# tlk00/BitMagic

Measured on AMD Instinct MI355X. Metric: Gbits/s + % HBM roofline, 256-way fused AND+COUNT on 1B-bit vectors, higher is better.
Workload: dtype u64; 1 GPU; aggregator pipeline combine_and_sub counts-only: 256-way AND+COUNT, 256 x 1000000000-bit vectors in total, data set A (common 10% OR noise 10%: no early exit); vectors=256, bits_per_vector=1000000000, density_q16=6554, blocks_per_vector=15259, blocks_per_rank=15259, hbm_resident_bytes=32279432448

## Files before the change

bitmagic_amd/csrc/bmx_device.h:

```cpp
#pragma once
#include <hip/hip_runtime.h>
#include <stdint.h>

typedef uint8_t  u8;
typedef uint16_t u16;
typedef uint32_t u32;
typedef uint64_t u64;

#define GMETA(e) ((u32)((e) >> 48) & 0x1FFFu)
#define GMETA_NONE 0xFFFFFFFFu
#define BMX_DESC_KIND(d) ((u32)((d) & 3ull))
#define BMX_DESC_PTR(d)  ((d) & ~3ull)

typedef u32 u32x4 __attribute__((ext_vector_type(4)));
typedef const __attribute__((address_space(1))) u32x4* gcptr4;
typedef __attribute__((address_space(1))) u32x4* gptr4;
typedef const __attribute__((address_space(1))) u16* gcptr16;

template <int ROWS> struct Part { u32x4 r[ROWS]; };
typedef Part<8> Blk;

__device__ __forceinline__ gcptr4 as_gc4(u64 addr) { return (gcptr4)(uintptr_t)addr; }
__device__ __forceinline__ gcptr4 as_gc4(const void* p) { return (gcptr4)(uintptr_t)p; }
__device__ __forceinline__ gptr4 as_g4(void* p) { return (gptr4)(uintptr_t)p; }
__device__ __forceinline__ gcptr16 as_gc16(u64 addr) { return (gcptr16)(uintptr_t)(addr & 0x0000FFFFFFFFFFFFull); }

__device__ __forceinline__ u32 lane_id() { return threadIdx.x & 63u; }

__device__ __forceinline__ u64 uniform64(u64 v)
{
    u32 lo = __builtin_amdgcn_readfirstlane((u32)v);
    u32 hi = __builtin_amdgcn_readfirstlane((u32)(v >> 32));
    return ((u64)hi << 32) | lo;
}
__device__ __forceinline__ u32 uniform32(u32 v) { return __builtin_amdgcn_readfirstlane(v); }

__device__ __forceinline__ u32 wave_sum(u32 v)
{
#pragma unroll
    for (int o = 32; o > 0; o >>= 1) v += __shfl_xor(v, o, 64);
    return v;
}

__device__ __forceinline__ u32 wave_scan_incl(u32 v, u32 )
{
    v += (u32)__builtin_amdgcn_update_dpp(0, (int)v, 0x111, 0xf, 0xf, false);
    v += (u32)__builtin_amdgcn_update_dpp(0, (int)v, 0x112, 0xf, 0xf, false);
    v += (u32)__builtin_amdgcn_update_dpp(0, (int)v, 0x114, 0xf, 0xf, false);
    v += (u32)__builtin_amdgcn_update_dpp(0, (int)v, 0x118, 0xf, 0xf, false);
    v += (u32)__builtin_amdgcn_update_dpp(0, (int)v, 0x142, 0xa, 0xf, false);
    v += (u32)__builtin_amdgcn_update_dpp(0, (int)v, 0x143, 0xc, 0xf, false);
    return v;
}

template <int ROWS, bool NT>
__device__ __forceinline__ void part_load(Part<ROWS>& b, gcptr4 p, u32 lane)
{
#pragma unroll
    for (int i = 0; i < ROWS; ++i) {
        if constexpr (NT) b.r[i] = __builtin_nontemporal_load(p + i * 64 + lane);
        else b.r[i] = p[i * 64 + lane];
    }
}
template <int ROWS>
__device__ __forceinline__ bool part_is_zero(const Part<ROWS>& b)
{
    u32 v = 0;
#pragma unroll
    for (int i = 0; i < ROWS; ++i) v |= b.r[i].x | b.r[i].y | b.r[i].z | b.r[i].w;
    return __ballot(v != 0u) == 0ull;
}
template <int ROWS>
__device__ __forceinline__ bool part_is_ones(const Part<ROWS>& b)
{
    u32 v = ~0u;
#pragma unroll
    for (int i = 0; i < ROWS; ++i) v &= b.r[i].x & b.r[i].y & b.r[i].z & b.r[i].w;
    return __ballot(v != ~0u) == 0ull;
}

__device__ __forceinline__ void blk_load(Blk& b, gcptr4 p, u32 lane)
{
#pragma unroll
    for (int i = 0; i < 8; ++i) b.r[i] = p[i * 64 + lane];
}
__device__ __forceinline__ void blk_store(const Blk& b, gptr4 p, u32 lane)
{
#pragma unroll
    for (int i = 0; i < 8; ++i) p[i * 64 + lane] = b.r[i];
}
__device__ __forceinline__ void blk_fill(Blk& b, u32 v)
{
#pragma unroll
    for (int i = 0; i < 8; ++i) b.r[i] = (u32x4)(v);
}
__device__ __forceinline__ void blk_and(Blk& a, const Blk& b)
{
#pragma unroll
    for (int i = 0; i < 8; ++i) a.r[i] &= b.r[i];
}
__device__ __forceinline__ void blk_andn(Blk& a, const Blk& b)
{
#pragma unroll
    for (int i = 0; i < 8; ++i) a.r[i] &= ~b.r[i];
}
__device__ __forceinline__ void blk_or(Blk& a, const Blk& b)
{
#pragma unroll
    for (int i = 0; i < 8; ++i) a.r[i] |= b.r[i];
}
__device__ __forceinline__ void blk_xor(Blk& a, const Blk& b)
{
#pragma unroll
    for (int i = 0; i < 8; ++i) a.r[i] ^= b.r[i];
}
__device__ __forceinline__ void blk_op(int op, Blk& a, const Blk& b)
{
    switch (op) { case 0: blk_and(a, b); break; case 1: blk_or(a, b); break;
                  case 2: blk_xor(a, b); break; default: blk_andn(a, b); break; }
}
__device__ __forceinline__ u32 blk_lane_or(const Blk& b)
{
    u32 v = 0;
#pragma unroll
    for (int i = 0; i < 8; ++i) v |= b.r[i].x | b.r[i].y | b.r[i].z | b.r[i].w;
    return v;
}
__device__ __forceinline__ u32 blk_lane_and(const Blk& b)
{
    u32 v = ~0u;
#pragma unroll
    for (int i = 0; i < 8; ++i) v &= b.r[i].x & b.r[i].y & b.r[i].z & b.r[i].w;
    return v;
}
// ... 604 lines not shown
```

bitmagic_amd/csrc/bmx_kernels6.h:

```cpp
#pragma once
#include "bmx_kernels5.h"


#define COLL_FLAG_FULL 1u
#define COLL_FLAG_NULL 2u
#define COLL_FLAG_BIT  4u
#define COLL_NGAP(f) ((f) >> 8)

typedef const __attribute__((address_space(1))) u64* coll_gc64;
typedef const __attribute__((address_space(1))) u32* coll_gc32;

__device__ __forceinline__ u32 coll_runs_of(u32 meta, u32 polarity)
{
    u32 len = meta >> 1, s = meta & 1u;
    u32 ones = s ? (len + 1u) >> 1 : len >> 1;
    return polarity ? ones : len - ones;
}

__global__ __launch_bounds__(256)
void k_coll_count(const u64* const* __restrict__ descs, const u32* __restrict__ nblk, u32 n, u32 ncols, u32 polarity,
                  u32* __restrict__ pre, u32* __restrict__ cnt, u32* __restrict__ flags)
{
    u32 c = blockIdx.x * blockDim.x + threadIdx.x;
    if (c >= ncols) return;
// ... 114 lines not shown
                for (int k = 0; k < 4; ++k) ns += (4u * q + (u32)k < m_cnt && p.start[k] == p.end[k]) ? 1u : 0u;
            }
        }
#pragma unroll
        for (u32 o = 1; o < (u32)L; o <<= 1) ns += __shfl_xor(ns, o, 64);
        if (in && t == 0) sgl[(size_t)i * ncols + c] = ns;
        else if (!in && t == 0 && c < ncols) sgl[(size_t)i * ncols + c] = 0u;
    }
}

__global__ __launch_bounds__(256)
void k_coll_prefix_singles(u32* __restrict__ sgl, u32 n, u32 ncols, const u32* __restrict__ cnt, u32* __restrict__ cnt_s, u32* __restrict__ words)
{
    const u32 c = blockIdx.x * blockDim.x + threadIdx.x;
    if (c >= ncols) return;
    u32 run = 0;
    for (u32 i = 0; i < n; ++i) { const u32 t = sgl[(size_t)i * ncols + c]; sgl[(size_t)i * ncols + c] = run; run += t; }
    cnt_s[c] = run;
    const u32 nm = cnt[c] - run;
    words[c] = ((nm + 3u) & ~3u) + (((run + 7u) & ~7u) >> 1);
}

template <int L>
__global__ __launch_bounds__(256)
void k_coll_scatter_split(const u64* const* __restrict__ descs, const u32* __restrict__ nblk, u32 ncols,
                          const u32* __restrict__ pre , const u32* __restrict__ pre_s ,
                          const u32* __restrict__ cnt, const u32* __restrict__ cnt_s, const u64* __restrict__ off, u32* __restrict__ runs)
{
    const u32 i = blockIdx.x;
    const u32 t = threadIdx.x % L;
    const u32 nb_i = nblk[i];
    const u32 lane = threadIdx.x & 63u, last = (lane & ~((u32)L - 1u)) + (u32)L - 1u;
    const u64* __restrict__ di = descs[i];
    auto dload = [&](u32 by) -> u64 { const u32 c = by * (256u / L) + threadIdx.x / L; return (c < ncols && c < nb_i) ? di[c] : 0ull; };
    u64 dn = dload(blockIdx.y * COLL_YT);
    for (u32 by = blockIdx.y * COLL_YT; by < (blockIdx.y + 1u) * COLL_YT; ++by) {
        if (by * (256u / L) >= ncols) break;
        const u32 c = by * (256u / L) + threadIdx.x / L;
        const u64 d = dn;
        dn = dload(by + 1u);
        if (DESC_K(d) != K_GAP) continue;
        const u32 meta = GMETA(d), len = meta >> 1, s = meta & 1u;
        const u32 m_cnt = coll_runs_of(meta, 1u);
        if (!m_cnt) continue;
        const u32 nchunks = (len + 1u + 7u) >> 3;
        gcptr4 g4 = as_gc4(DESC_P(d));
        const u64 base = off[c];
        const u32 ps = pre_s[(size_t)i * ncols + c], pt = pre[(size_t)i * ncols + c] & 0x3FFFFFFFu;
        const u32 nm_col = cnt[c] - cnt_s[c];
        u32* om = runs + base + (pt - ps);
        u16* os = reinterpret_cast<u16*>(runs + base + ((nm_col + 3u) & ~3u)) + ps;
        for (u32 q0 = 0; q0 < nchunks; q0 += (u32)L) {
            const u32 q = q0 + t;
            const bool have = q < nchunks;
            const u32x4 x = have ? g4[q] : (u32x4)(0u);
            const u32 nx = (have && q + 1u < nchunks) ? g4[q + 1u].x : 0xFFFFFFFFu;
            CollPairs p;
            coll_chunk_pairs(x, nx, s, q, p);
            bool valid[4], single[4];
            u32 ns = 0, nm = 0;
#pragma unroll
            for (int k = 0; k < 4; ++k) {
                valid[k] = have && 4u * q + (u32)k < m_cnt;
                single[k] = valid[k] && p.start[k] == p.end[k];
                ns += single[k] ? 1u : 0u; nm += (valid[k] && !single[k]) ? 1u : 0u;
            }
            u32 is = ns, im = nm;
#pragma unroll
            for (u32 o = 1; o < (u32)L; o <<= 1) {
                const u32 a = __shfl_up(is, o, 64), b = __shfl_up(im, o, 64);
                if (t >= o) { is += a; im += b; }
            }
            u16* ws = os + (is - ns); u32* wm = om + (im - nm);
#pragma unroll
            for (int k = 0; k < 4; ++k) {
                if (single[k]) *ws++ = (u16)p.start[k];
                else if (valid[k]) *wm++ = p.start[k] | (p.end[k] << 16);
            }
            os += __shfl(is, (int)last, 64); om += __shfl(im, (int)last, 64);
        }
    }
}

__device__ __forceinline__ void coll_apply_run(u32 r, bool valid, u32* U, int* D, u32& any_long)
{
    u32 s = r & 0xFFFFu, e = r >> 16;
    u32 ws = s >> 5, we = e >> 5;
    u32 lo = ~0u << (s & 31u), hi = ~0u >> (31u - (e & 31u));
    bool same = ws == we;
    if (valid) atomicOr(&U[ws], same ? (lo & hi) : lo);
    if (valid && !same) {
        atomicOr(&U[we], hi);
        if (we - ws > 1u) { atomicAdd(&D[ws + 1u], 1); atomicSub(&D[we], 1); any_long = 1u; }
    }
}

template <int WG, bool PF, bool CW = false>
__device__ __forceinline__ u32 coll_apply_bag(const u32* __restrict__ runs, u64 off, u32 cnt, u32* U, int* D, u32 tid, bool diag_loads_only = false)
{
    gcptr4 p = as_gc4(runs + off);
    const u32 nq = (cnt + 3u) >> 2;
    u32 any_long = 0u;
    if (!nq) return 0u;
    constexpr u32 JS = CW ? 64u : (u32)WG;
    const u32 first = CW ? (tid >> 6) * 256u + (tid & 63u) : tid;
    auto fetch = [&](u32x4 (&v)[4], u32 q0) {
#pragma unroll
        for (u32 j = 0; j < 4; ++j) { u32 q = q0 + j * JS; v[j] = __builtin_nontemporal_load(&p[q < nq ? q : nq - 1u]); }
    };
    auto apply = [&](const u32x4 (&v)[4], u32 q0) {
#ifdef BMX_DIAG
        if (diag_loads_only) {
            u32 t = 0;
            for (u32 j = 0; j < 4; ++j) t |= v[j].x | v[j].y | v[j].z | v[j].w;
            if (t == 0x12345u) U[tid] = t;
            return;
        }
#endif
#pragma unroll
        for (u32 j = 0; j < 4; ++j) {
            u32 q = q0 + j * JS;
            bool in = q < nq;
            u32 e0 = q * 4u;
            coll_apply_run(v[j].x, in && e0 < cnt, U, D, any_long);
            coll_apply_run(v[j].y, in && e0 + 1u < cnt, U, D, any_long);
            coll_apply_run(v[j].z, in && e0 + 2u < cnt, U, D, any_long);
            coll_apply_run(v[j].w, in && e0 + 3u < cnt, U, D, any_long);
        }
    };
    if constexpr (PF) {
        u32x4 a[4], b[4];
        const u32 rounds = (nq + 4u * WG - 1u) / (4u * WG);
        fetch(a, first);
        for (u32 r = 0; r < rounds; r += 2u) {
            fetch(b, first + (r + 1u) * 4u * WG);
            apply(a, first + r * 4u * WG);
            fetch(a, first + (r + 2u) * 4u * WG);
            apply(b, first + (r + 1u) * 4u * WG);
        }
    } else {
        const u32 rounds = (nq + 4u * WG - 1u) / (4u * WG);
        for (u32 r = 0; r < rounds; ++r) { u32x4 v[4]; fetch(v, first + r * 4u * WG); apply(v, first + r * 4u * WG); }
    }
    return any_long;
}

template <int WG, bool CW>
__device__ __forceinline__ void coll_apply_singles(const u32* __restrict__ words, u64 off_words, u32 ns, u32* U, u32 tid)
{
    gcptr4 p = as_gc4(words + off_words);
    const u32 nq = (ns + 7u) >> 3;
    if (!nq) return;
    constexpr u32 JS = CW ? 64u : (u32)WG;
    const u32 first = CW ? (tid >> 6) * 256u + (tid & 63u) : tid;
    const u32 rounds = (nq + 4u * WG - 1u) / (4u * WG);
    for (u32 r = 0; r < rounds; ++r) {
        u32x4 v[4];
        const u32 q0 = first + r * 4u * WG;
#pragma unroll
        for (u32 j = 0; j < 4; ++j) { u32 q = q0 + j * JS; v[j] = __builtin_nontemporal_load(&p[q < nq ? q : nq - 1u]); }
#pragma unroll
        for (u32 j = 0; j < 4; ++j) {
            const u32 q = q0 + j * JS;
            const u32 e0 = q * 8u;
            const u32 w4[4] = {v[j].x, v[j].y, v[j].z, v[j].w};
#pragma unroll
            for (u32 t = 0; t < 4; ++t) {
                const u32 lo = w4[t] & 0xFFFFu, hi = w4[t] >> 16;
                if (q < nq && e0 + 2u * t < ns) atomicOr(&U[lo >> 5], 1u << (lo & 31u));
                if (q < nq && e0 + 2u * t + 1u < ns) atomicOr(&U[hi >> 5], 1u << (hi & 31u));
            }
        }
    }
}

template <int WG>
__device__ __forceinline__ void coll_fold(u32* U, int* D, int* sm, u32 tid)
{
    constexpr u32 W = 2048u / WG;
    const u32 lane = tid & 63u, wave = tid >> 6;
    int d[W]; int sum = 0;
#pragma unroll
    for (u32 k = 0; k < W; k += 4u) {
        u32x4 t = *reinterpret_cast<u32x4*>(&D[tid * W + k]);
        d[k] = (int)t.x; d[k + 1] = (int)t.y; d[k + 2] = (int)t.z; d[k + 3] = (int)t.w;
        *reinterpret_cast<u32x4*>(&D[tid * W + k]) = (u32x4)(0u);
    }
#pragma unroll
    for (u32 k = 0; k < W; ++k) sum += d[k];
    int incl = (int)wave_scan_incl((u32)sum, lane);
    if (lane == 63) sm[wave] = incl;
    __syncthreads();
    int running = incl - sum;
#pragma unroll
    for (u32 i = 0; i < WG / 64u; ++i) if (i < wave) running += sm[i];
#pragma unroll
    for (u32 k = 0; k < W; ++k) { running += d[k]; if (running > 0) U[tid * W + k] = ~0u; }
    __syncthreads();
}

__global__ __launch_bounds__(256)
void k_vec_alg_bytes(const u64* __restrict__ desc, u32 nblocks, u64* __restrict__ out)
{
    u32 nb = blockIdx.x * blockDim.x + threadIdx.x;
    u32 b = 0;
    if (nb < nblocks) {
        u64 d = desc[nb];
        u32 k = DESC_K(d);
        b = k == K_BIT ? 8192u : (k == K_GAP ? 2u * ((GMETA(d) >> 1) + 1u) : 0u);
    }
    b = wave_sum(b);
    if ((threadIdx.x & 63u) == 0 && b) atomicAdd(reinterpret_cast<unsigned long long*>(out), (unsigned long long)b);
}

enum { COLL_OR = 0, COLL_AND_STORE = 1, COLL_AND_COUNT = 2 };

template <int MODE, int WG, bool PF = false, bool CW = false>
__global__ __launch_bounds__(WG)
void k_coll_apply(const u32* __restrict__ runs, const u64* __restrict__ off, const u32* __restrict__ cnt,
                  const u32* __restrict__ flags, u32 ncols_a,
                  const u32* __restrict__ s_runs, const u64* __restrict__ s_off, const u32* __restrict__ s_cnt,
                  const u32* __restrict__ s_flags, u32 ncols_s,
                  u32 col_base, u32 ncols, int opt_compress, u64* __restrict__ counts,
                  uint4* __restrict__ slab, u64* __restrict__ desc, BlockStat* __restrict__ st, u32 hint_from, u32 hint_to,
                  FoldOut kinds ,
                  const u32* __restrict__ a_cnt_s ,
                  const u32* __restrict__ s_cnt_s )
{
    __shared__ __attribute__((aligned(16))) u32 U[2048];
    __shared__ __attribute__((aligned(16))) int D[2048];
    __shared__ int sm[WG / 64];
    __shared__ u32 s_long;
    __shared__ u32 part[WG / 64];
    const u32 tid = threadIdx.x, lane = tid & 63u, wave = tid >> 6;
#ifdef BMX_DIAG
    const int diag = opt_compress & 1536;
    opt_compress &= 1;
#endif
    const u32 c = col_base + blockIdx.x;
    if (c >= ncols) return;
    if (MODE != COLL_OR && (c < hint_from || c >= hint_to)) {
        if (MODE == COLL_AND_STORE && wave == 0) store_trivial(K_NULL, c, desc, st, lane);
        return;
    }
    const u32 fl = c < ncols_a ? uniform32(flags[c]) : (MODE == COLL_OR ? 0u : COLL_FLAG_NULL);
    const u32 n_ent = c < ncols_a ? uniform32(cnt[c]) : 0u;
    if (MODE == COLL_OR) {
        if ((fl & COLL_FLAG_FULL) || COLL_NGAP(fl) == 0u) {
            const u32 k = (fl & COLL_FLAG_FULL) ? (u32)K_FULL : (u32)K_NULL;
            if (wave == 0) store_trivial(k, c, desc, st, lane);
            if (kinds.slots) kind_fanin_fold(wave == 0 ? k : 4u, kinds, lane, wave);
            return;
        }
    } else {
        const u32 sfl = (s_flags && c < ncols_s) ? uniform32(s_flags[c]) : 0u;
        if ((fl & COLL_FLAG_NULL) || (sfl & COLL_FLAG_FULL)) {
            if (MODE == COLL_AND_STORE && wave == 0) store_trivial(K_NULL, c, desc, st, lane);
            return;
        }
    }
    constexpr u32 W = 2048u / WG;
#pragma unroll
    for (u32 k = 0; k < W; k += 4u) {
        *reinterpret_cast<u32x4*>(&U[tid * W + k]) = (u32x4)(0u);
        *reinterpret_cast<u32x4*>(&D[tid * W + k]) = (u32x4)(0u);
    }
    if (tid == 0) s_long = 0u;
    __syncthreads();
    const u64 a_off = uniform64(off[c < ncols_a ? c : 0u]);
    const u32 a_ns = (a_cnt_s && c < ncols_a) ? uniform32(a_cnt_s[c]) : 0u;
    const u32 a_nm = n_ent - a_ns;
#ifdef BMX_DIAG
    u32 al = coll_apply_bag<WG, PF, CW>(runs, a_off, a_nm, U, D, tid, (diag & 512) != 0);
    if (diag & 1024) return;
#else
    u32 al = coll_apply_bag<WG, PF, CW>(runs, a_off, a_nm, U, D, tid);
#endif
    if (a_ns) coll_apply_singles<WG, CW>(runs, a_off + ((a_nm + 3u) & ~3u), a_ns, U, tid);
    if (al) s_long = 1u;
    __syncthreads();
    if (s_long) coll_fold<WG>(U, D, sm, tid);
    if (MODE == COLL_OR) {
        u32 kind = 4u;
        if (wave == 0) {
            Blk b; blk_from_lds(b, U, lane);
            kind = store_result_mode(b, c, opt_compress ? ST_OPT : ST_FORCE_BIT, slab, desc, st, lane);
        }
        if (kinds.slots) kind_fanin_fold(kind, kinds, lane, wave);
        return;
    }
    u32 acc[W];
#pragma unroll
    for (u32 k = 0; k < W; ++k) acc[k] = ~U[tid * W + k];
    const u32 s_ent = (s_cnt && c < ncols_s) ? uniform32(s_cnt[c]) : 0u;
    if (s_ent) {
        __syncthreads();
#pragma unroll
        for (u32 k = 0; k < W; k += 4u) *reinterpret_cast<u32x4*>(&U[tid * W + k]) = (u32x4)(0u);
        if (tid == 0) s_long = 0u;
        __syncthreads();
        const u64 so = uniform64(s_off[c]);
        const u32 s_ns = s_cnt_s ? uniform32(s_cnt_s[c]) : 0u, s_nm = s_ent - s_ns;
        u32 sl = coll_apply_bag<WG, PF, CW>(s_runs, so, s_nm, U, D, tid);
        if (s_ns) coll_apply_singles<WG, CW>(s_runs, so + ((s_nm + 3u) & ~3u), s_ns, U, tid);
        if (sl) s_long = 1u;
        __syncthreads();
        if (s_long) coll_fold<WG>(U, D, sm, tid);
#pragma unroll
        for (u32 k = 0; k < W; ++k) acc[k] &= ~U[tid * W + k];
    }
    if (MODE == COLL_AND_COUNT) {
        u32 pc = 0;
#pragma unroll
        for (u32 k = 0; k < W; ++k) pc += (u32)__popc(acc[k]);
        pc = wave_sum(pc);
        if (lane == 0) part[wave] = pc;
        __syncthreads();
        if (tid == 0) {
            u32 t = 0;
#pragma unroll
            for (u32 i = 0; i < WG / 64u; ++i) t += part[i];
            if (t) atomicAdd(reinterpret_cast<unsigned long long*>(&counts[0]), (unsigned long long)t);
        }
        return;
    }
    __syncthreads();
#pragma unroll
    for (u32 k = 0; k < W; ++k) U[tid * W + k] = acc[k];
    __syncthreads();
    if (wave == 0) { Blk b; blk_from_lds(b, U, lane); store_result(b, c, 1, slab, desc, st, lane); }
}

__global__ __launch_bounds__(256)
void k_block_counts(const u64* __restrict__ desc, u32 nblocks, u32* __restrict__ bcount)
{
    u32 lane = lane_id(), wave = threadIdx.x >> 6;
    u32 nb = uniform32(blockIdx.x * 4u + wave);
    if (nb >= nblocks) return;
    u64 d = uniform64(desc[nb]);
    u32 k = DESC_K(d), c = 0;
    if (k == K_FULL) c = 65536u;
    else if (k == K_BIT) { Blk b; blk_load(b, as_gc4(DESC_P(d)), lane); c = wave_sum(blk_lane_popcount(b)); }
    else if (k == K_GAP) c = wave_sum(gap_lane_popcount(as_gc16(DESC_P(d)), lane, GMETA(d)));
    if (lane == 0) bcount[nb] = c;
}

template <typename T>
__device__ __forceinline__ void emit_word_bits(u32 w, u64 base, T* __restrict__ out, u64& off)
{
    while (w) { u32 b = (u32)__builtin_ctz(w); out[off++] = (T)(base + b); w &= w - 1u; }
}

template <typename T>
__global__ __launch_bounds__(256)
void k_expand_indices(const u64* __restrict__ desc, u32 nblocks, const u64* __restrict__ rcount, T* __restrict__ out, u64 cap, u64 pos_base)
{
    __shared__ u32 lds[4 * 2048];
    u32 lane = lane_id(), wave = threadIdx.x >> 6;
    u32 nb = uniform32(blockIdx.x * 4u + wave);
    if (nb >= nblocks) return;
    u64 d = uniform64(desc[nb]);
    u32 k = DESC_K(d);
    if (k == K_NULL) return;
    u64 first = nb ? rcount[nb - 1u] : 0ull;
    u64 last = rcount[nb];
    if (last > cap) return;
    u64 bit0 = pos_base + ((u64)nb << 16);
    if (k == K_FULL) {
        for (u32 i = lane; i < 65536u; i += 64u) out[first + i] = (T)(bit0 + i);
        return;
    }
    Blk b;
    blk_from_desc(d, b, lds + wave * 2048u, lane);
    u64 row_off = first;
#pragma unroll
    for (int i = 0; i < 8; ++i) {
        u32 c = (u32)__popc(b.r[i].x) + (u32)__popc(b.r[i].y) + (u32)__popc(b.r[i].z) + (u32)__popc(b.r[i].w);
        u32 incl = wave_scan_incl(c, lane);
        u32 tot = uniform32(__shfl(incl, 63, 64));
        u64 off = row_off + (incl - c);
        u64 wb = bit0 + ((u64)((u32)i * 256u + lane * 4u) << 5);
        emit_word_bits<T>(b.r[i].x, wb, out, off);
        emit_word_bits<T>(b.r[i].y, wb + 32u, out, off);
        emit_word_bits<T>(b.r[i].z, wb + 64u, out, off);
        emit_word_bits<T>(b.r[i].w, wb + 96u, out, off);
        row_off += tot;
    }
}

__device__ __forceinline__ u32 select_in_word(u32 w, u32 k)
// ... 634 lines not shown
```

bitmagic_amd/csrc/bmx_kernels9.h:

```cpp
#pragma once
#include "bmx_kernels8.h"


enum { AR_COUNT = 0, AR_STORE = 1 };

#ifdef BMX_DIAG
__device__ __forceinline__ void ar_apply_run_diag(u32 r, bool valid, u32* U, int* D, int diag, u32 lane, u32& sink)
{
    const u32 s = (u32)(u16)((u16)r + (u16)1u), e = r >> 16;
    u32 ws = s >> 5, we = r >> 21;
    const u32 ml = ~0u << (s & 31u), mh = ~(~1u << (e & 31u));
    const bool same = ws == we;
    if (diag & 4) { if (valid) { sink ^= (same ? (ml & mh) : ml) + ws; if (!same) sink ^= mh + we; } return; }
    if (valid) {
        atomicOr(&U[lane], same ? (ml & mh) : ml);
        if (!same) { atomicOr(&U[lane + 64u], mh); atomicAdd(&D[lane + 128u], 1); atomicSub(&D[lane + 192u], 1); }
    }
}
#endif
__device__ __forceinline__ void ar_apply_run(u32 r, bool valid, u32* U, int* D)
{
    const u32 s = (u32)(u16)((u16)r + (u16)1u), e = r >> 16;
    const u32 ws = s >> 5, we = r >> 21;
    const u32 ml = ~0u << (s & 31u), mh = ~(~1u << (e & 31u));
    const bool same = ws == we;
    if (valid) {
        atomicOr(&U[ws], same ? (ml & mh) : ml);
        if (!same) { atomicOr(&U[we], mh); atomicAdd(&D[ws + 1u], 1); atomicSub(&D[we], 1); }
    }
}

template <int WG, int DEPTH, bool NT>
__device__ __forceinline__ void ar_union_list(const u64* __restrict__ list_back, u32 n, u32 want, u32* U, int* D, u32 lane, u32 wave, u64 dummy, int diag = 0)
{
    constexpr u32 NW = (u32)WG / 64u;
    const u32 mine = wave < n ? (n - wave + NW - 1u) / NW : 0u;
    for (u32 b0 = 0; b0 < mine; b0 += 64u) {
        const u32 nb = mine - b0 < 64u ? mine - b0 : 64u;
        u64 ent = 0ull;
        if (lane < nb) ent = *(list_back - (size_t)(wave + NW * (b0 + lane)));
        const u32 elo = (u32)ent, ehi = (u32)(ent >> 32);
        const u32 nch_l = lane < nb ? (((ehi >> 17) & 0xFFFu) + 8u) >> 3 : 0u;
        const u32 incl = wave_scan_incl(nch_l, lane);
        const u32 cum = incl - nch_l;
        const u32 T = (u32)__builtin_amdgcn_readlane((int)incl, 63);
        const u32 npieces = (T + 63u) >> 6;
        u32x4 c[DEPTH];
        u32 cs[DEPTH], ms[DEPTH];
        u32 iq = 0u, jn = 0u;
        auto issue = [&](int k) {
            const bool have = iq < npieces;
            const u32 base = iq << 6;
            const u32 jprev = jn;
            u64 M = 0ull;
            if (have) {
                while (jn < nb) {
                    const u32 cj = (u32)__builtin_amdgcn_readlane((int)cum, (int)jn);
                    if (cj >= base + 64u) break;
                    M |= 1ull << (cj - base);
                    ++jn;
                }
            }
            const u64 Ms = M >> 1;
            const u32 o = (u32)__builtin_amdgcn_mbcnt_hi((u32)(Ms >> 32), __builtin_amdgcn_mbcnt_lo((u32)Ms, jprev - 1u + (u32)(M & 1ull)));
            const u32 g = base + lane;
            const u32 gc = g < T ? g : T - 1u;
            const int oa = (int)(o << 2);
            const u32 plo = (u32)__builtin_amdgcn_ds_bpermute(oa, (int)elo);
            const u32 phi = (u32)__builtin_amdgcn_ds_bpermute(oa, (int)ehi);
            const u32 pcu = (u32)__builtin_amdgcn_ds_bpermute(oa, (int)cum);
            const u32 ci = gc - pcu;
            u64 a = ((u64)plo | ((u64)(phi & 0xFFFFu) << 32)) + ((u64)ci << 4);
            if (!have) a = dummy;
            c[k] = NT ? __builtin_nontemporal_load((gcptr4)(uintptr_t)a) : *(gcptr4)(uintptr_t)a;
            cs[k] = (have && g < T) ? ci : 0x0FFFFFFFu;
            ms[k] = phi;
            ++iq;
        };
#pragma unroll
        for (int k = 0; k < DEPTH; ++k) issue(k);
        u32 carry = 0u;
        for (u32 q0 = 0; q0 < npieces; q0 += (u32)DEPTH) {
#pragma unroll
            for (int k = 0; k < DEPTH; ++k) {
                if (q0 + (u32)k < npieces) {
                    const u32 ci = cs[k];
                    const u32 len = (ms[k] >> 17) & 0xFFFu;
                    const bool odd = ((ms[k] >> 16) & 1u) == want;
                    const u32 pw = (u32)__builtin_amdgcn_update_dpp((int)carry, (int)c[k].w, 0x138 , 0xf, 0xf, false);
                    carry = (u32)__builtin_amdgcn_readlane((int)c[k].w, 63);
                    const u32 sel = odd ? 0x07060504u : 0x05040302u;
                    const u32 x0 = ci == 0u ? (c[k].x | 0xFFFFu) : c[k].x;
                    const u32 d[5] = {pw, x0, c[k].y, c[k].z, c[k].w};
                    const int lim = (int)len - (int)(8u * ci + (odd ? 1u : 0u));
                    const int lim0 = (ci == 0u && !odd) ? -1 : lim;
#ifdef BMX_DIAG
                    if (diag & 1) { if ((d[0] ^ d[1] ^ d[2] ^ d[3] ^ d[4] ^ sel ^ (u32)lim0) == 0x12345679u) U[lane] = 1u; }
                    else if (diag & 12) {
                        u32 sink = 0u;
                        ar_apply_run_diag(__builtin_amdgcn_perm(d[1], d[0], sel), lim0 >= 0, U, D, diag, lane, sink);
                        ar_apply_run_diag(__builtin_amdgcn_perm(d[2], d[1], sel), lim >= 2, U, D, diag, lane, sink);
                        ar_apply_run_diag(__builtin_amdgcn_perm(d[3], d[2], sel), lim >= 4, U, D, diag, lane, sink);
                        ar_apply_run_diag(__builtin_amdgcn_perm(d[4], d[3], sel), lim >= 6, U, D, diag, lane, sink);
                        if (sink == 0x12345679u) U[lane] = 1u;
                    } else
#endif
                    {
                        ar_apply_run(__builtin_amdgcn_perm(d[1], d[0], sel), lim0 >= 0, U, D);
                        ar_apply_run(__builtin_amdgcn_perm(d[2], d[1], sel), lim >= 2, U, D);
                        ar_apply_run(__builtin_amdgcn_perm(d[3], d[2], sel), lim >= 4, U, D);
                        ar_apply_run(__builtin_amdgcn_perm(d[4], d[3], sel), lim >= 6, U, D);
                    }
                }
                issue(k);
            }
        }
    }
}

template <int MODE, int WG, int DEPTH, bool NT>
__device__ __forceinline__ void ar_item(u32 item, u32* U, int* D, int* sm, u32* part, const u64* __restrict__ dmat, const u32* __restrict__ row_off, const u32* __restrict__ and_n,
                    const u32* __restrict__ sub_n, u32 col_stride, u32 ngroups, u32 col_from, u32 nitems, int xcd_swz,
                    u64* __restrict__ counts, uint4* __restrict__ slab, u64* __restrict__ desc, BlockStat* __restrict__ st,
                    u32 hint_from, u32 hint_to, int diag)
{
    const u32 tid = threadIdx.x, lane = tid & 63u, wave = uniform32(tid >> 6);
    const u32 ci = item / ngroups, g = item - ci * ngroups;
    const u32 col = col_from + ci;
    if (MODE == AR_STORE && (col < hint_from || col >= hint_to)) { if (wave == 0) store_trivial(K_NULL, col, desc, st, lane); return; }
    const u64* row = dmat + (size_t)col * col_stride + uniform32(row_off[g]);
    const u64 hdr = uniform64(row[0]), flags = uniform64(row[1]);
    if (flags & ROW_EMPTY) { if (MODE == AR_STORE && wave == 0) store_trivial(K_NULL, col, desc, st, lane); return; }
    if (flags & ROW_FULL) {
        if (MODE == AR_STORE) { if (wave == 0) store_trivial(K_FULL, col, desc, st, lane); }
        else if (tid == 0) atomicAdd(reinterpret_cast<unsigned long long*>(&counts[g]), 65536ull);
        return;
    }
    const u32 nga = (u32)((hdr >> 16) & 0xFFFFu), ngs = (u32)(hdr >> 48);
    const u32 na = uniform32(and_n[g]), ns = uniform32(sub_n[g]);
    constexpr u32 W = 2048u / (u32)WG;
#pragma unroll
    for (u32 k = 0; k < W; k += 4u) {
        *reinterpret_cast<u32x4*>(&U[tid * W + k]) = (u32x4)(0u);
        *reinterpret_cast<u32x4*>(&D[tid * W + k]) = (u32x4)(0u);
    }
    __syncthreads();
    const u64 dummy = (u64)(uintptr_t)dmat;
    if (nga) ar_union_list<WG, DEPTH, NT>(row + 2 + na - 1u, nga, 0u, U, D, lane, wave, dummy, diag);
#ifdef BMX_DIAG
    if (diag & 2) return;
#endif
    __syncthreads();
    if (nga) coll_fold<WG>(U, D, sm, tid);
    u32 acc[W];
#pragma unroll
    for (u32 k = 0; k < W; ++k) acc[k] = ~U[tid * W + k];
    if (ngs) {
        __syncthreads();
#pragma unroll
        for (u32 k = 0; k < W; k += 4u) *reinterpret_cast<u32x4*>(&U[tid * W + k]) = (u32x4)(0u);
        __syncthreads();
        ar_union_list<WG, DEPTH, NT>(row + 2 + na + ns - 1u, ngs, 1u, U, D, lane, wave, dummy, diag);
        __syncthreads();
        coll_fold<WG>(U, D, sm, tid);
#pragma unroll
        for (u32 k = 0; k < W; ++k) acc[k] &= ~U[tid * W + k];
    }
    if (MODE == AR_COUNT) {
        u32 pc = 0;
#pragma unroll
        for (u32 k = 0; k < W; ++k) pc += (u32)__popc(acc[k]);
        pc = wave_sum(pc);
        if (lane == 0) part[wave] = pc;
        __syncthreads();
        if (tid == 0) {
            u32 t = 0;
#pragma unroll
            for (u32 i = 0; i < (u32)WG / 64u; ++i) t += part[i];
            if (t) atomicAdd(reinterpret_cast<unsigned long long*>(&counts[g]), (unsigned long long)t);
        }
        return;
    }
    __syncthreads();
#pragma unroll
    for (u32 k = 0; k < W; ++k) U[tid * W + k] = acc[k];
    __syncthreads();
    if (wave == 0) { Blk b; blk_from_lds(b, U, lane); store_result(b, col, 1, slab, desc, st, lane); }
}

template <int MODE, int WG, int DEPTH, bool NT>
__global__ __launch_bounds__(WG)
void k_agg_and_rows(const u64* __restrict__ dmat, const u32* __restrict__ row_off, const u32* __restrict__ and_n,
                    const u32* __restrict__ sub_n, u32 col_stride, u32 ngroups, u32 col_from, u32 nitems, int xcd_swz,
                    u64* __restrict__ counts, uint4* __restrict__ slab, u64* __restrict__ desc, BlockStat* __restrict__ st,
                    u32 hint_from, u32 hint_to, int diag, u32 ipw)
{
    __shared__ __attribute__((aligned(16))) u32 U[2048];
    __shared__ __attribute__((aligned(16))) int D[2048];
    __shared__ int sm[WG / 64];
    __shared__ u32 part[WG / 64];
    const u32 b = xcd_swz ? xcd_remap(blockIdx.x, gridDim.x) : blockIdx.x;
    for (u32 k = 0; k < ipw; ++k) {
        const u32 item = b * ipw + k;
        if (item >= nitems) return;
        if (k) __syncthreads();
        ar_item<MODE, WG, DEPTH, NT>(item, U, D, sm, part, dmat, row_off, and_n, sub_n, col_stride, ngroups, col_from, nitems, xcd_swz, counts, slab, desc, st,
                                     hint_from, hint_to, diag);
    }
}

struct LimitTables {
    const u32* row_off; const u32* and_n; const u32* sub_n;
    u32* ro; u32* an; u32* sn;
    const CollGroup* cg_in; CollGroup* cg_out;
    const u32* gmask_in; const u32* gskip_in; u32* gmask_out; u32* gskip_out; u32 nchunks;
};

__global__ __launch_bounds__(1024)
void k_limit_step(u64* __restrict__ totals, const u64* __restrict__ cc, const u32* __restrict__ active_in , u32 n_in,
                  u64 limit, u32 win_end, u32* __restrict__ stop, u32* __restrict__ active_out, LimitTables t,
                  u32* __restrict__ n_active_dev, u64* __restrict__ n_active_host)
{
    __shared__ u32 wsum[16];
    __shared__ u32 base;
    const u32 tid = threadIdx.x, lane = tid & 63u, wave = tid >> 6;
    if (tid == 0) base = 0u;
    __syncthreads();
    for (u32 i0 = 0; i0 < n_in; i0 += 1024u) {
        const u32 i = i0 + tid;
        bool keep = false; u32 g = 0u;
        if (i < n_in) {
            g = active_in ? active_in[i] : i;
            const u64 c = totals[g] + cc[i];
            totals[g] = c;
            keep = c < limit;
            if (!keep && stop[g] == 0xFFFFFFFFu) stop[g] = win_end;
        }
        const u64 m = __ballot(keep);
        if (lane == 0) wsum[wave] = (u32)__popcll(m);
        __syncthreads();
        u32 off = base;
        for (u32 w = 0; w < wave; ++w) off += wsum[w];
        if (keep) {
            const u32 pos = off + (u32)__builtin_amdgcn_mbcnt_hi((u32)(m >> 32), __builtin_amdgcn_mbcnt_lo((u32)m, 0u));
            active_out[pos] = g;
            t.ro[pos] = t.row_off[g]; t.an[pos] = t.and_n[g]; t.sn[pos] = t.sub_n[g];
            if (t.cg_in) t.cg_out[pos] = t.cg_in[g];
            if (t.gmask_in) {
                for (u32 k = 0; k < t.nchunks; ++k) t.gmask_out[(size_t)pos * t.nchunks + k] = t.gmask_in[(size_t)g * t.nchunks + k];
                t.gskip_out[pos] = t.gskip_in[g];
            }
        }
        __syncthreads();
        if (tid == 0) { u32 s = 0; for (u32 w = 0; w < 16u; ++w) s += wsum[w]; base += s; }
        __syncthreads();
    }
    if (tid == 0) { *n_active_dev = base; *n_active_host = (u64)base; }
}

__global__ __launch_bounds__(256)
void k_pipe_null_rows(u64* __restrict__ dmat, u32 ncols, u32 col_stride, u32 null_off)
{
    const u32 c = blockIdx.x * blockDim.x + threadIdx.x;
    if (c >= ncols) return;
    u64* row = dmat + (size_t)c * col_stride + null_off;
    row[0] = 0ull; row[1] = ROW_EMPTY;
}

__global__ __launch_bounds__(256)
void k_limit_null(u64* __restrict__ totals, const u64* __restrict__ cc, u32 ng, u64 limit, u32 null_off,
                  u32* __restrict__ ro, CollGroup* __restrict__ cg, u32* __restrict__ gskip, u64* __restrict__ out )
{
    const u32 g = blockIdx.x * blockDim.x + threadIdx.x;
    if (g >= ng) return;
    const u64 c = totals[g] + cc[g];
    totals[g] = c;
    if (c >= limit) {
        ro[g] = null_off;
        if (cg) cg[g] = CollGroup{0u, 0u, 0u, 0u};
        if (gskip) gskip[g] = 1u;
    }
    if (out) out[g] = c;
}
```

Before: 55290 Gbit/s.

## Replace run difference-array fold with per-word max-end coverage scan

Multi-word runs are no longer applied as an atomic OR at the end word plus atomic add/sub into a difference array. Each run now records only its end bit with an atomicMax into a per-start-word array E. The fold step ORs each recorded end-word mask and fills interior words with a prefix max scan (DPP max plus per-wave maxima). This cuts the LDS atomics per long run from four to two. Separately, launch bounds get waves-per-SIMD hints for several aggregator configurations, which changes register allocation and occupancy.

```diff
diff --git a/bitmagic_amd/csrc/bmx_device.h b/bitmagic_amd/csrc/bmx_device.h
--- a/bitmagic_amd/csrc/bmx_device.h
+++ b/bitmagic_amd/csrc/bmx_device.h
@@ -50,6 +50,17 @@
     v += (u32)__builtin_amdgcn_update_dpp(0, (int)v, 0x118, 0xf, 0xf, false);
     v += (u32)__builtin_amdgcn_update_dpp(0, (int)v, 0x142, 0xa, 0xf, false);
     v += (u32)__builtin_amdgcn_update_dpp(0, (int)v, 0x143, 0xc, 0xf, false);
+    return v;
+}
+__device__ __forceinline__ u32 wave_scan_incl_max(u32 v)
+{
+    auto mx = [](u32 a, u32 b) { return a > b ? a : b; };
+    v = mx(v, (u32)__builtin_amdgcn_update_dpp(0, (int)v, 0x111, 0xf, 0xf, false));
+    v = mx(v, (u32)__builtin_amdgcn_update_dpp(0, (int)v, 0x112, 0xf, 0xf, false));
+    v = mx(v, (u32)__builtin_amdgcn_update_dpp(0, (int)v, 0x114, 0xf, 0xf, false));
+    v = mx(v, (u32)__builtin_amdgcn_update_dpp(0, (int)v, 0x118, 0xf, 0xf, false));
+    v = mx(v, (u32)__builtin_amdgcn_update_dpp(0, (int)v, 0x142, 0xa, 0xf, false));
+    v = mx(v, (u32)__builtin_amdgcn_update_dpp(0, (int)v, 0x143, 0xc, 0xf, false));
     return v;
 }
 
diff --git a/bitmagic_amd/csrc/bmx_kernels6.h b/bitmagic_amd/csrc/bmx_kernels6.h
--- a/bitmagic_amd/csrc/bmx_kernels6.h
+++ b/bitmagic_amd/csrc/bmx_kernels6.h
@@ -220,21 +220,18 @@
     }
 }
 
-__device__ __forceinline__ void coll_apply_run(u32 r, bool valid, u32* U, int* D, u32& any_long)
+__device__ __forceinline__ void coll_apply_run(u32 r, bool valid, u32* U, u32* E, u32& any_long)
 {
     u32 s = r & 0xFFFFu, e = r >> 16;
     u32 ws = s >> 5, we = e >> 5;
     u32 lo = ~0u << (s & 31u), hi = ~0u >> (31u - (e & 31u));
     bool same = ws == we;
     if (valid) atomicOr(&U[ws], same ? (lo & hi) : lo);
-    if (valid && !same) {
-        atomicOr(&U[we], hi);
-        if (we - ws > 1u) { atomicAdd(&D[ws + 1u], 1); atomicSub(&D[we], 1); any_long = 1u; }
-    }
+    if (valid && !same) { atomicMax(&E[ws], e); any_long = 1u; }
 }
 
 template <int WG, bool PF, bool CW = false>
-__device__ __forceinline__ u32 coll_apply_bag(const u32* __restrict__ runs, u64 off, u32 cnt, u32* U, int* D, u32 tid, bool diag_loads_only = false)
+__device__ __forceinline__ u32 coll_apply_bag(const u32* __restrict__ runs, u64 off, u32 cnt, u32* U, u32* E, u32 tid, bool diag_loads_only = false)
 {
     gcptr4 p = as_gc4(runs + off);
     const u32 nq = (cnt + 3u) >> 2;
@@ -260,10 +257,10 @@
             u32 q = q0 + j * JS;
             bool in = q < nq;
             u32 e0 = q * 4u;
-            coll_apply_run(v[j].x, in && e0 < cnt, U, D, any_long);
-            coll_apply_run(v[j].y, in && e0 + 1u < cnt, U, D, any_long);
-            coll_apply_run(v[j].z, in && e0 + 2u < cnt, U, D, any_long);
-            coll_apply_run(v[j].w, in && e0 + 3u < cnt, U, D, any_long);
+            coll_apply_run(v[j].x, in && e0 < cnt, U, E, any_long);
+            coll_apply_run(v[j].y, in && e0 + 1u < cnt, U, E, any_long);
+            coll_apply_run(v[j].z, in && e0 + 2u < cnt, U, E, any_long);
+            coll_apply_run(v[j].w, in && e0 + 3u < cnt, U, E, any_long);
         }
     };
     if constexpr (PF) {
@@ -313,27 +310,31 @@
 }
 
 template <int WG>
-__device__ __forceinline__ void coll_fold(u32* U, int* D, int* sm, u32 tid)
+__device__ __forceinline__ void coll_fold(u32* U, u32* E, u32* sm, u32 tid)
 {
     constexpr u32 W = 2048u / WG;
     const u32 lane = tid & 63u, wave = tid >> 6;
-    int d[W]; int sum = 0;
+    u32 ew[W]; u32 mx = 0u;
 #pragma unroll
     for (u32 k = 0; k < W; k += 4u) {
-        u32x4 t = *reinterpret_cast<u32x4*>(&D[tid * W + k]);
-        d[k] = (int)t.x; d[k + 1] = (int)t.y; d[k + 2] = (int)t.z; d[k + 3] = (int)t.w;
-        *reinterpret_cast<u32x4*>(&D[tid * W + k]) = (u32x4)(0u);
-    }
-#pragma unroll
-    for (u32 k = 0; k < W; ++k) sum += d[k];
-    int incl = (int)wave_scan_incl((u32)sum, lane);
+        u32x4 t = *reinterpret_cast<u32x4*>(&E[tid * W + k]);
+        ew[k] = t.x; ew[k + 1] = t.y; ew[k + 2] = t.z; ew[k + 3] = t.w;
+        *reinterpret_cast<u32x4*>(&E[tid * W + k]) = (u32x4)(0u);
+    }
+#pragma unroll
+    for (u32 k = 0; k < W; ++k) {
+        if (ew[k]) atomicOr(&U[ew[k] >> 5], ~(~1u << (ew[k] & 31u)));
+        ew[k] >>= 5;
+        mx = ew[k] > mx ? ew[k] : mx;
+    }
+    const u32 incl = wave_scan_incl_max(mx);
     if (lane == 63) sm[wave] = incl;
     __syncthreads();
-    int running = incl - sum;
-#pragma unroll
-    for (u32 i = 0; i < WG / 64u; ++i) if (i < wave) running += sm[i];
-#pragma unroll
-    for (u32 k = 0; k < W; ++k) { running += d[k]; if (running > 0) U[tid * W + k] = ~0u; }
+    u32 running = (u32)__builtin_amdgcn_update_dpp(0, (int)incl, 0x138 , 0xf, 0xf, false);
+#pragma unroll
+    for (u32 i = 0; i < WG / 64u; ++i) if (i < wave) running = sm[i] > running ? sm[i] : running;
+#pragma unroll
+    for (u32 k = 0; k < W; ++k) { if (running > tid * W + k) U[tid * W + k] = ~0u; running = ew[k] > running ? ew[k] : running; }
     __syncthreads();
 }
 
@@ -366,8 +367,8 @@
                   const u32* __restrict__ s_cnt_s )
 {
     __shared__ __attribute__((aligned(16))) u32 U[2048];
-    __shared__ __attribute__((aligned(16))) int D[2048];
-    __shared__ int sm[WG / 64];
+    __shared__ __attribute__((aligned(16))) u32 E[2048];
+    __shared__ u32 sm[WG / 64];
     __shared__ u32 s_long;
     __shared__ u32 part[WG / 64];
     const u32 tid = threadIdx.x, lane = tid & 63u, wave = tid >> 6;
@@ -401,7 +402,7 @@
 #pragma unroll
     for (u32 k = 0; k < W; k += 4u) {
         *reinterpret_cast<u32x4*>(&U[tid * W + k]) = (u32x4)(0u);
-        *reinterpret_cast<u32x4*>(&D[tid * W + k]) = (u32x4)(0u);
+        *reinterpret_cast<u32x4*>(&E[tid * W + k]) = (u32x4)(0u);
     }
     if (tid == 0) s_long = 0u;
     __syncthreads();
@@ -409,15 +410,15 @@
     const u32 a_ns = (a_cnt_s && c < ncols_a) ? uniform32(a_cnt_s[c]) : 0u;
     const u32 a_nm = n_ent - a_ns;
 #ifdef BMX_DIAG
-    u32 al = coll_apply_bag<WG, PF, CW>(runs, a_off, a_nm, U, D, tid, (diag & 512) != 0);
+    u32 al = coll_apply_bag<WG, PF, CW>(runs, a_off, a_nm, U, E, tid, (diag & 512) != 0);
     if (diag & 1024) return;
 #else
-    u32 al = coll_apply_bag<WG, PF, CW>(runs, a_off, a_nm, U, D, tid);
+    u32 al = coll_apply_bag<WG, PF, CW>(runs, a_off, a_nm, U, E, tid);
 #endif
     if (a_ns) coll_apply_singles<WG, CW>(runs, a_off + ((a_nm + 3u) & ~3u), a_ns, U, tid);
     if (al) s_long = 1u;
     __syncthreads();
-    if (s_long) coll_fold<WG>(U, D, sm, tid);
+    if (s_long) coll_fold<WG>(U, E, sm, tid);
     if (MODE == COLL_OR) {
         u32 kind = 4u;
         if (wave == 0) {
@@ -439,11 +440,11 @@
         __syncthreads();
         const u64 so = uniform64(s_off[c]);
         const u32 s_ns = s_cnt_s ? uniform32(s_cnt_s[c]) : 0u, s_nm = s_ent - s_ns;
-        u32 sl = coll_apply_bag<WG, PF, CW>(s_runs, so, s_nm, U, D, tid);
+        u32 sl = coll_apply_bag<WG, PF, CW>(s_runs, so, s_nm, U, E, tid);
         if (s_ns) coll_apply_singles<WG, CW>(s_runs, so + ((s_nm + 3u) & ~3u), s_ns, U, tid);
         if (sl) s_long = 1u;
         __syncthreads();
-        if (s_long) coll_fold<WG>(U, D, sm, tid);
+        if (s_long) coll_fold<WG>(U, E, sm, tid);
 #pragma unroll
         for (u32 k = 0; k < W; ++k) acc[k] &= ~U[tid * W + k];
     }
diff --git a/bitmagic_amd/csrc/bmx_kernels9.h b/bitmagic_amd/csrc/bmx_kernels9.h
--- a/bitmagic_amd/csrc/bmx_kernels9.h
+++ b/bitmagic_amd/csrc/bmx_kernels9.h
@@ -5,33 +5,33 @@
 enum { AR_COUNT = 0, AR_STORE = 1 };
 
 #ifdef BMX_DIAG
-__device__ __forceinline__ void ar_apply_run_diag(u32 r, bool valid, u32* U, int* D, int diag, u32 lane, u32& sink)
+__device__ __forceinline__ void ar_apply_run_diag(u32 r, bool valid, u32* U, u32* E, int diag, u32 lane, u32& sink)
 {
     const u32 s = (u32)(u16)((u16)r + (u16)1u), e = r >> 16;
-    u32 ws = s >> 5, we = r >> 21;
+    const u32 ws = s >> 5;
     const u32 ml = ~0u << (s & 31u), mh = ~(~1u << (e & 31u));
-    const bool same = ws == we;
-    if (diag & 4) { if (valid) { sink ^= (same ? (ml & mh) : ml) + ws; if (!same) sink ^= mh + we; } return; }
+    const bool same = ws == r >> 21;
+    if (diag & 4) { if (valid) { sink ^= (same ? (ml & mh) : ml) + ws; if (!same) sink ^= e + ws; } return; }
     if (valid) {
         atomicOr(&U[lane], same ? (ml & mh) : ml);
-        if (!same) { atomicOr(&U[lane + 64u], mh); atomicAdd(&D[lane + 128u], 1); atomicSub(&D[lane + 192u], 1); }
+        if (!same) atomicMax(&E[lane], e);
     }
 }
 #endif
-__device__ __forceinline__ void ar_apply_run(u32 r, bool valid, u32* U, int* D)
+__device__ __forceinline__ void ar_apply_run(u32 r, bool valid, u32* U, u32* E)
 {
     const u32 s = (u32)(u16)((u16)r + (u16)1u), e = r >> 16;
-    const u32 ws = s >> 5, we = r >> 21;
+    const u32 ws = s >> 5;
     const u32 ml = ~0u << (s & 31u), mh = ~(~1u << (e & 31u));
-    const bool same = ws == we;
+    const bool same = ws == r >> 21;
     if (valid) {
         atomicOr(&U[ws], same ? (ml & mh) : ml);
-        if (!same) { atomicOr(&U[we], mh); atomicAdd(&D[ws + 1u], 1); atomicSub(&D[we], 1); }
+        if (!same) atomicMax(&E[ws], e);
     }
 }
 
 template <int WG, int DEPTH, bool NT>
-__device__ __forceinline__ void ar_union_list(const u64* __restrict__ list_back, u32 n, u32 want, u32* U, int* D, u32 lane, u32 wave, u64 dummy, int diag = 0)
+__device__ __forceinline__ void ar_union_list(const u64* __restrict__ list_back, u32 n, u32 want, u32* U, u32* E, u32 lane, u32 wave, u64 dummy, int diag = 0)
 {
     constexpr u32 NW = (u32)WG / 64u;
     const u32 mine = wave < n ? (n - wave + NW - 1u) / NW : 0u;
@@ -98,18 +98,18 @@
                     if (diag & 1) { if ((d[0] ^ d[1] ^ d[2] ^ d[3] ^ d[4] ^ sel ^ (u32)lim0) == 0x12345679u) U[lane] = 1u; }
                     else if (diag & 12) {
                         u32 sink = 0u;
-                        ar_apply_run_diag(__builtin_amdgcn_perm(d[1], d[0], sel), lim0 >= 0, U, D, diag, lane, sink);
-                        ar_apply_run_diag(__builtin_amdgcn_perm(d[2], d[1], sel), lim >= 2, U, D, diag, lane, sink);
-                        ar_apply_run_diag(__builtin_amdgcn_perm(d[3], d[2], sel), lim >= 4, U, D, diag, lane, sink);
-                        ar_apply_run_diag(__builtin_amdgcn_perm(d[4], d[3], sel), lim >= 6, U, D, diag, lane, sink);
+                        ar_apply_run_diag(__builtin_amdgcn_perm(d[1], d[0], sel), lim0 >= 0, U, E, diag, lane, sink);
+                        ar_apply_run_diag(__builtin_amdgcn_perm(d[2], d[1], sel), lim >= 2, U, E, diag, lane, sink);
+                        ar_apply_run_diag(__builtin_amdgcn_perm(d[3], d[2], sel), lim >= 4, U, E, diag, lane, sink);
+                        ar_apply_run_diag(__builtin_amdgcn_perm(d[4], d[3], sel), lim >= 6, U, E, diag, lane, sink);
                         if (sink == 0x12345679u) U[lane] = 1u;
                     } else
 #endif
                     {
-                        ar_apply_run(__builtin_amdgcn_perm(d[1], d[0], sel), lim0 >= 0, U, D);
-                        ar_apply_run(__builtin_amdgcn_perm(d[2], d[1], sel), lim >= 2, U, D);
-                        ar_apply_run(__builtin_amdgcn_perm(d[3], d[2], sel), lim >= 4, U, D);
-                        ar_apply_run(__builtin_amdgcn_perm(d[4], d[3], sel), lim >= 6, U, D);
+                        ar_apply_run(__builtin_amdgcn_perm(d[1], d[0], sel), lim0 >= 0, U, E);
+                        ar_apply_run(__builtin_amdgcn_perm(d[2], d[1], sel), lim >= 2, U, E);
+                        ar_apply_run(__builtin_amdgcn_perm(d[3], d[2], sel), lim >= 4, U, E);
+                        ar_apply_run(__builtin_amdgcn_perm(d[4], d[3], sel), lim >= 6, U, E);
                     }
                 }
                 issue(k);
@@ -119,7 +119,7 @@
 }
 
 template <int MODE, int WG, int DEPTH, bool NT>
-__device__ __forceinline__ void ar_item(u32 item, u32* U, int* D, int* sm, u32* part, const u64* __restrict__ dmat, const u32* __restrict__ row_off, const u32* __restrict__ and_n,
+__device__ __forceinline__ void ar_item(u32 item, u32* U, u32* E, u32* sm, u32* part, const u64* __restrict__ dmat, const u32* __restrict__ row_off, const u32* __restrict__ and_n,
                     const u32* __restrict__ sub_n, u32 col_stride, u32 ngroups, u32 col_from, u32 nitems, int xcd_swz,
                     u64* __restrict__ counts, uint4* __restrict__ slab, u64* __restrict__ desc, BlockStat* __restrict__ st,
                     u32 hint_from, u32 hint_to, int diag)
@@ -142,16 +142,16 @@
 #pragma unroll
     for (u32 k = 0; k < W; k += 4u) {
         *reinterpret_cast<u32x4*>(&U[tid * W + k]) = (u32x4)(0u);
-        *reinterpret_cast<u32x4*>(&D[tid * W + k]) = (u32x4)(0u);
+        *reinterpret_cast<u32x4*>(&E[tid * W + k]) = (u32x4)(0u);
     }
     __syncthreads();
     const u64 dummy = (u64)(uintptr_t)dmat;
-    if (nga) ar_union_list<WG, DEPTH, NT>(row + 2 + na - 1u, nga, 0u, U, D, lane, wave, dummy, diag);
+    if (nga) ar_union_list<WG, DEPTH, NT>(row + 2 + na - 1u, nga, 0u, U, E, lane, wave, dummy, diag);
 #ifdef BMX_DIAG
     if (diag & 2) return;
 #endif
     __syncthreads();
-    if (nga) coll_fold<WG>(U, D, sm, tid);
+    if (nga) coll_fold<WG>(U, E, sm, tid);
     u32 acc[W];
 #pragma unroll
     for (u32 k = 0; k < W; ++k) acc[k] = ~U[tid * W + k];
@@ -160,9 +160,9 @@
 #pragma unroll
         for (u32 k = 0; k < W; k += 4u) *reinterpret_cast<u32x4*>(&U[tid * W + k]) = (u32x4)(0u);
         __syncthreads();
-        ar_union_list<WG, DEPTH, NT>(row + 2 + na + ns - 1u, ngs, 1u, U, D, lane, wave, dummy, diag);
-        __syncthreads();
-        coll_fold<WG>(U, D, sm, tid);
+        ar_union_list<WG, DEPTH, NT>(row + 2 + na + ns - 1u, ngs, 1u, U, E, lane, wave, dummy, diag);
+        __syncthreads();
+        coll_fold<WG>(U, E, sm, tid);
 #pragma unroll
         for (u32 k = 0; k < W; ++k) acc[k] &= ~U[tid * W + k];
     }
@@ -188,23 +188,30 @@
     if (wave == 0) { Blk b; blk_from_lds(b, U, lane); store_result(b, col, 1, slab, desc, st, lane); }
 }
 
+constexpr int ar_waves_per_simd(int mode, int wg, int depth)
+{
+    if (mode == AR_STORE) return wg >= 256 && depth <= 2 ? 5 : 0;
+    if (wg == 256 && depth == 4) return 8;
+    if (wg == 128 && depth == 8) return 5;
+    return 0;
+}
 template <int MODE, int WG, int DEPTH, bool NT>
-__global__ __launch_bounds__(WG)
+__global__ __launch_bounds__(WG, ar_waves_per_simd(MODE, WG, DEPTH))
 void k_agg_and_rows(const u64* __restrict__ dmat, const u32* __restrict__ row_off, const u32* __restrict__ and_n,
                     const u32* __restrict__ sub_n, u32 col_stride, u32 ngroups, u32 col_from, u32 nitems, int xcd_swz,
                     u64* __restrict__ counts, uint4* __restrict__ slab, u64* __restrict__ desc, BlockStat* __restrict__ st,
                     u32 hint_from, u32 hint_to, int diag, u32 ipw)
 {
     __shared__ __attribute__((aligned(16))) u32 U[2048];
-    __shared__ __attribute__((aligned(16))) int D[2048];
-    __shared__ int sm[WG / 64];
+    __shared__ __attribute__((aligned(16))) u32 E[2048];
+    __shared__ u32 sm[WG / 64];
     __shared__ u32 part[WG / 64];
     const u32 b = xcd_swz ? xcd_remap(blockIdx.x, gridDim.x) : blockIdx.x;
     for (u32 k = 0; k < ipw; ++k) {
         const u32 item = b * ipw + k;
         if (item >= nitems) return;
         if (k) __syncthreads();
-        ar_item<MODE, WG, DEPTH, NT>(item, U, D, sm, part, dmat, row_off, and_n, sub_n, col_stride, ngroups, col_from, nitems, xcd_swz, counts, slab, desc, st,
+        ar_item<MODE, WG, DEPTH, NT>(item, U, E, sm, part, dmat, row_off, and_n, sub_n, col_stride, ngroups, col_from, nitems, xcd_swz, counts, slab, desc, st,
                                      hint_from, hint_to, diag);
     }
 }
```

Result: no change. 55170 Gbit/s (-0.2%).
